# zwu88/TANTE

Measured on NVIDIA B200. Metric: training_samples_per_s, higher is better.
Workload: dtype bf16

## Files before the change

include/tante_b200.h:

```cpp
#ifndef TANTE_B200_H_
#define TANTE_B200_H_

#include <stddef.h>
#include <stdint.h>

#ifdef __cplusplus
extern "C" {
#endif

#if defined(__GNUC__)
#define TANTE_API __attribute__((visibility("default")))
#else
#define TANTE_API
#endif

#define TANTE_OK 0
#define TANTE_ERR_INVALID 1
#define TANTE_ERR_CUDA 2
#define TANTE_ERR_STATE 3
#define TANTE_ERR_NOMEM 4

#define TANTE_MAX_ORDER 8
#define TANTE_MAX_LAYERS 32

// ... 54 lines not shown
                        int32_t n_cap, float* frames, float* R_t, int32_t* n_host, void* stream);
TANTE_API int tante_backward(tante_handle_t h, int32_t slot, const float* input, const float* grad_frames,
                   int32_t n_frames, const float* grad_Rt, float* grad_input, float* grad_params, void* stream);

TANTE_API int tante_train_forward_win(tante_handle_t h, int32_t slot, const float* const* frame_ptrs,
                                      const int64_t* frame_bstride, int32_t B, float out_T, int32_t n_cap, float* frames,
                                      int64_t frames_bstride, float* R_t, int32_t* n_host, void* stream);
TANTE_API int tante_backward_win(tante_handle_t h, int32_t slot, const float* grad_frames, int64_t gf_bstride, int32_t n_frames,
                                 const float* grad_Rt, float* const* grad_frame_ptrs, const int64_t* grad_bstride,
                                 float* grad_params, void* stream);

TANTE_API int tante_train_forward_hist(tante_handle_t h, int32_t slot, const float* input, float* pred, int64_t pred_bstride,
                                       int32_t* cursor, int32_t B, float out_T, int32_t n_cap, int32_t n_steps, float* R_t,
                                       int32_t* ns, int32_t* steps, int32_t* n_active, void* stream);
TANTE_API int tante_backward_hist(tante_handle_t h, int32_t slot, float* grad_pred, int64_t gp_bstride, const float* grad_Rt,
                                  float* grad_input, float* grad_params, void* stream);

TANTE_API int tante_debug_stage(tante_handle_t h, const char* stage, float* dst, int64_t cap, int64_t* numel,
                      void* stream);
TANTE_API int64_t tante_launch_count(tante_handle_t h);

TANTE_API int tante_bench_head(tante_handle_t h, const float* u, float* frames, int32_t B, int32_t n_frames,
                     int32_t iters, float* ms_out, void* stream);

TANTE_API int tante_profile(tante_handle_t h, int32_t enable);
TANTE_API int tante_profile_read(tante_handle_t h, double* gemm_ms, double* gemm_flops, int64_t* gemm_launches);
TANTE_API int tante_profile_read_class(tante_handle_t h, int32_t cls, double* ms, double* flops, double* bytes,
                                       int64_t* launches);

TANTE_API int tante_mse_cl(const float* y, const float* ref, int32_t B, int32_t nf, int32_t n_use, int32_t D, int64_t HW,
                 int32_t n_ref, int32_t f0, float scale, const float* gout, float* loss_sum, float* grad_y, void* stream);

TANTE_API int tante_metric_moments(const float* x, const float* y, int64_t BT, int64_t HW, int32_t C, double* out,
                                   void* stream);

TANTE_API int tante_comm_unique_id(void* id128);
TANTE_API int tante_comm_init(tante_handle_t h, const void* id128, int32_t nranks, int32_t rank);
TANTE_API int tante_allreduce_grads(tante_handle_t h, float* grad, void* comm, void* stream);
TANTE_API int tante_optimizer_step(tante_handle_t h, float* grad, float* exp_avg, float* exp_avg_sq, float lr, float beta1,
                                   float beta2, float eps, float weight_decay, int64_t step, int32_t clip_mode, float clip,
                                   float grad_scale, double* grad_sumsq, void* stream);

TANTE_API int tante_test_gemm(int32_t use_tc, int32_t epi, const void* A, const void* W, const float* bias,
                    const float* resid, void* C, int32_t out_bf16, int32_t M, int32_t N, int32_t K,
                    int32_t iters, const float* ln_gamma, const float* ln_beta, void* ln_out, void* stream);

TANTE_API int tante_test_block_tail(const void* att, const void* Wo, const void* W1, const void* W2, const float* vec7,
                                    const float* x_in, float* x_out, void* ln_out, float* x_mid, void* ln2, void* hpre,
                                    void* hact, int32_t M, int32_t iters, void* stream);

TANTE_API int tante_test_wgrad(int32_t use_tc, const void* A, const void* B, float* C, float* bias, int64_t M, int32_t N,
                     int32_t K, int32_t iters, void* stream);

#ifdef __cplusplus
}
#endif
#endif
```

tante_b200/_abi.py:

```python
from __future__ import annotations

import ctypes as C
import os

_HERE = os.path.dirname(os.path.abspath(__file__))
LIB_PATH = os.path.join(_HERE, "lib", "libtante_b200.so")

TANTE_MAX_ORDER = 8
TANTE_MAX_LAYERS = 32
PREC_FP32 = 0
PREC_BF16 = 1


class TanteConfig(C.Structure):
    _fields_ = [
        ("in_T", C.c_int32), ("n_fields", C.c_int32), ("H", C.c_int32), ("W", C.c_int32),
        ("taylor_order", C.c_int32), ("n_head", C.c_int32), ("embed_dim", C.c_int32),
        ("patch_scale", C.c_int32), ("deg", C.c_int32), ("output_length", C.c_int32),
        ("frame_interval", C.c_float), ("precision", C.c_int32),
        ("n_layers", C.c_int32 * TANTE_MAX_ORDER),
        ("axes", (C.c_char * TANTE_MAX_LAYERS) * TANTE_MAX_ORDER),
        ("enc_dec_fno", C.c_int32), ("modes1", C.c_int32), ("modes2", C.c_int32),
        ("mlp_hidden", C.c_int32),
        ("expanded_channel", C.c_int32), ("mlp_hidden_c", C.c_int32),
# ... 11 lines not shown
SIGNATURES = {
    "tante_last_error": (C.c_char_p, []),
    "tante_version": (C.c_int, []),
    "tante_create": (C.c_int, [C.POINTER(TanteConfig), C.c_int, C.POINTER(C.c_void_p)]),
    "tante_destroy": (C.c_int, [C.c_void_p]),
    "tante_reserve": (C.c_int, [C.c_void_p, C.c_int32, C.c_int32, C.c_int32]),
    "tante_workspace_bytes": (C.c_int64, [C.c_void_p]),
    "tante_param_count": (C.c_int32, [C.c_void_p]),
    "tante_param_name": (C.c_char_p, [C.c_void_p, C.c_int32]),
    "tante_param_numel": (C.c_int64, [C.c_void_p, C.c_int32]),
    "tante_bind_param": (C.c_int, [C.c_void_p, C.c_char_p, C.c_void_p, C.c_void_p, C.c_int64]),
    "tante_pack_params": (C.c_int, [C.c_void_p, C.c_void_p]),
    "tante_forward": (C.c_int, [C.c_void_p, C.c_void_p, C.c_int32, C.c_float, C.c_int32, C.c_int32,
                                C.c_void_p, C.c_void_p, C.c_void_p, C.POINTER(C.c_int32), C.c_void_p]),
    "tante_rollout": (C.c_int, [C.c_void_p, C.c_void_p, C.c_int32, C.c_int32, C.c_float, C.c_int32,
                                C.c_void_p, C.c_void_p, C.c_void_p, C.c_void_p, C.c_int32, C.c_void_p]),
    "tante_debug_stage": (C.c_int, [C.c_void_p, C.c_char_p, C.c_void_p, C.c_int64, C.POINTER(C.c_int64), C.c_void_p]),
    "tante_launch_count": (C.c_int64, [C.c_void_p]),
    "tante_profile": (C.c_int, [C.c_void_p, C.c_int32]),
    "tante_profile_read": (C.c_int, [C.c_void_p, C.POINTER(C.c_double), C.POINTER(C.c_double), C.POINTER(C.c_int64)]),
    "tante_profile_read_class": (C.c_int, [C.c_void_p, C.c_int32, C.POINTER(C.c_double), C.POINTER(C.c_double),
                                           C.POINTER(C.c_double), C.POINTER(C.c_int64)]),
    "tante_mse_cl": (C.c_int, [C.c_void_p, C.c_void_p, C.c_int32, C.c_int32, C.c_int32, C.c_int32, C.c_int64, C.c_int32,
                               C.c_int32, C.c_float, C.c_void_p, C.c_void_p, C.c_void_p, C.c_void_p]),
    "tante_test_block_tail": (C.c_int, [C.c_void_p] * 12 + [C.c_int32, C.c_int32, C.c_void_p]),
    "tante_metric_moments": (C.c_int, [C.c_void_p, C.c_void_p, C.c_int64, C.c_int64, C.c_int32, C.c_void_p, C.c_void_p]),
    "tante_test_gemm": (C.c_int, [C.c_int32, C.c_int32, C.c_void_p, C.c_void_p, C.c_void_p, C.c_void_p, C.c_void_p,
                                  C.c_int32, C.c_int32, C.c_int32, C.c_int32, C.c_int32, C.c_void_p, C.c_void_p, C.c_void_p,
                                  C.c_void_p]),
    "tante_comm_unique_id": (C.c_int, [C.c_void_p]),
    "tante_comm_init": (C.c_int, [C.c_void_p, C.c_void_p, C.c_int32, C.c_int32]),
    "tante_allreduce_grads": (C.c_int, [C.c_void_p, C.c_void_p, C.c_void_p, C.c_void_p]),
    "tante_optimizer_step": (C.c_int, [C.c_void_p, C.c_void_p, C.c_void_p, C.c_void_p, C.c_float, C.c_float, C.c_float,
                                       C.c_float, C.c_float, C.c_int64, C.c_int32, C.c_float, C.c_float, C.c_void_p,
                                       C.c_void_p]),
    "tante_set_dropout": (C.c_int, [C.c_void_p, C.c_float, C.c_uint64]),
    "tante_grad_numel": (C.c_int64, [C.c_void_p]),
    "tante_param_grad_offset": (C.c_int64, [C.c_void_p, C.c_int32]),
    "tante_train_forward": (C.c_int, [C.c_void_p, C.c_int32, C.c_void_p, C.c_int32, C.c_float, C.c_int32,
                                      C.c_void_p, C.c_void_p, C.POINTER(C.c_int32), C.c_void_p]),
    "tante_backward": (C.c_int, [C.c_void_p, C.c_int32, C.c_void_p, C.c_void_p, C.c_int32, C.c_void_p, C.c_void_p,
                                 C.c_void_p, C.c_void_p]),
    "tante_train_forward_win": (C.c_int, [C.c_void_p, C.c_int32, C.POINTER(C.c_void_p), C.POINTER(C.c_int64), C.c_int32, C.c_float,
                                          C.c_int32, C.c_void_p, C.c_int64, C.c_void_p, C.POINTER(C.c_int32), C.c_void_p]),
    "tante_backward_win": (C.c_int, [C.c_void_p, C.c_int32, C.c_void_p, C.c_int64, C.c_int32, C.c_void_p, C.POINTER(C.c_void_p),
                                     C.POINTER(C.c_int64), C.c_void_p, C.c_void_p]),
    "tante_train_forward_hist": (C.c_int, [C.c_void_p, C.c_int32, C.c_void_p, C.c_void_p, C.c_int64, C.c_void_p, C.c_int32,
                                           C.c_float, C.c_int32, C.c_int32, C.c_void_p, C.c_void_p, C.c_void_p, C.c_void_p,
                                           C.c_void_p]),
    "tante_backward_hist": (C.c_int, [C.c_void_p, C.c_int32, C.c_void_p, C.c_int64, C.c_void_p, C.c_void_p, C.c_void_p,
                                      C.c_void_p]),
    "tante_test_wgrad": (C.c_int, [C.c_int32, C.c_void_p, C.c_void_p, C.c_void_p, C.c_void_p, C.c_int64, C.c_int32,
                                   C.c_int32, C.c_int32, C.c_void_p]),
    "tante_bench_head": (C.c_int, [C.c_void_p, C.c_void_p, C.c_void_p, C.c_int32, C.c_int32, C.c_int32,
                                   C.POINTER(C.c_float), C.c_void_p]),
}

_lib = None


def load() -> C.CDLL:
    global _lib
    if _lib is not None:
        return _lib
    if not os.path.exists(LIB_PATH):
        raise ImportError(
            f"{LIB_PATH} not found: build it with `python -m tante_b200.build` (nvcc, sm_100a). "
            "tante_b200 has no fallback path.")
    lib = C.CDLL(LIB_PATH)
    for name, (res, args) in SIGNATURES.items():
        fn = getattr(lib, name)
        fn.restype = res
        fn.argtypes = args
    _lib = lib
    return lib


def check(code: int):
    if code != 0:
        raise TanteError(code, (load().tante_last_error() or b"").decode())
```

tante_b200/csrc/tante_abi.cu:

```cuda
#include <cuda_runtime.h>

#include <algorithm>
#include <cmath>
#include <cstdio>
#include <cstring>
#include <map>
#include <memory>
#include <stdexcept>
#include <string>
#include <vector>

#include "../../include/tante_b200.h"
#include "common.cuh"
#include "gemm_simt.cuh"
#include "gemm_tc.cuh"
#include "attention_mma.cuh"
#include "attention_flash.cuh"
#include "propagator_mma.cuh"
#include "propagator_bwd_mma.cuh"
#include "propagator_small.cuh"
#include "head_mma.cuh"
#include "kernels_simt.cuh"
#include "pack.cuh"
#include "backward.cuh"
// ... 1288 lines not shown
template <typename TA, int ACT>
void launch_act_fwd(tante_handle_s* h, const TA* pre, TA* out, long long n, cudaStream_t st) {
    act_fwd_kernel<TA, ACT><<<blocks_for(n / 4, 256), 256, 0, st>>>(pre, out, n / 4);
    CK(cudaGetLastError());
    h->launches++;
}
template <typename TA, int ACT>
void launch_act_bwd(tante_handle_s* h, TA* g, const TA* pre, long long n, cudaStream_t st) {
    act_bwd_kernel<TA, ACT><<<blocks_for(n / 4, 256), 256, 0, st>>>(g, pre, n / 4);
    CK(cudaGetLastError());
    h->launches++;
}
template <typename TA>
void launch_colsum(tante_handle_s* h, const TA* x, int ld, long long M, int N, float* out, cudaStream_t st) {
    const unsigned gx = (unsigned)((N + 127) / 128);
    unsigned gy = (unsigned)std::max<long long>(1, std::min<long long>((M + 255) / 256, (4LL * h->num_sms + gx - 1) / gx));
    colsum_kernel<TA><<<dim3(gx, gy), 256, 0, st>>>(x, ld, M, N, out);
    CK(cudaGetLastError());
    h->launches++;
}
template <typename TA>
void wgrad(tante_handle_s* h, const TA* A, int lda, const TA* Bm, int ldb, float* out, long long M, int N, int K,
           cudaStream_t st, float* bias_out = nullptr) {
    {
        ProfScope ps(h, st, 2.0 * (double)M * N * K, 2, (double)M * (N + K) * sizeof(TA));
        if constexpr (sizeof(TA) == 2) {
            if (wgrad_tc_supported(M, N, K, K, lda, ldb, K)) {
                CK(launch_wgrad_tc(A, lda, Bm, ldb, out, K, M, N, K, K, h->num_sms, st, bias_out));
                h->launches++;
                return;
            }
        }
        CK((launch_wgrad_simt<TA, TA>(A, lda, Bm, ldb, out, K, M, N, K, h->num_sms, st)));
        h->launches++;
    }
    if (bias_out) launch_colsum<TA>(h, A, lda, M, N, bias_out, st);
}
template <typename TA>
void wgrad_pad(tante_handle_s* h, const TA* A, int lda, int N, const TA* Bm, int ldb, int Kb, float* out, int ldc, int Kc,
               long long M, cudaStream_t st, float* bias_out = nullptr) {
    {
        ProfScope ps(h, st, 2.0 * (double)M * N * Kc, 2, (double)M * (N + Kb) * sizeof(TA));
        if constexpr (sizeof(TA) == 2) {
            if (wgrad_tc_supported(M, N, Kb, Kc, lda, ldb, ldc)) {
                CK(launch_wgrad_tc(A, lda, Bm, ldb, out, ldc, M, N, Kb, Kc, h->num_sms, st, bias_out));
                h->launches++;
                return;
            }
        }
        CK((launch_wgrad_simt<TA, TA>(A, lda, Bm, ldb, out, ldc, M, N, Kc, h->num_sms, st)));
        h->launches++;
    }
    if (bias_out) launch_colsum<TA>(h, A, lda, M, N, bias_out, st);
}
template <typename TA>
void gemm_dx(tante_handle_s* h, const TA* A, int lda, int64_t wT_off, TA* out, int ldc, int M, int N, int K, cudaStream_t st) {
    EpiParams ep; ep.bias = AF(h, h->zero_off);
    REQUIRE(N <= 8192, "input-gradient GEMM wider than the zero-bias vector");
    if (sizeof(TA) == 2 && K > 1024) {
        REQUIRE(ldc == N, "input-gradient GEMM: K not covered");
        if (h->kscratch.bytes < (size_t)M * N * 4) destroy_graphs(h);
        dev_alloc(h, h->kscratch, (size_t)M * N * 4);
        float* v = FP(h->kscratch);
        gemm_bigk_f32(h, reinterpret_cast<const __nv_bfloat16*>(A), lda, wT_off, v, M, N, K, AF(h, h->zero_off), st);
        convert_kernel<TA><<<blocks_for((long long)M * N / 4, 256), 256, 0, st>>>(v, out, (long long)M * N / 4);
        CK(cudaGetLastError());
        h->launches++;
        return;
    }
    gemm<TA>(h, EPI_BIAS, A, lda, wT_off, out, ldc, sizeof(TA) == 4, M, N, K, ep, st);
}

template <typename TA, int ACT>
void gemm_dx_act(tante_handle_s* h, const TA* A, int lda, int64_t wT_off, TA* out, const TA* pre, int M, int N, int K,
                 cudaStream_t st) {
    static const bool fuse = getenv("TANTE_FUSE_ACTGRAD") && atoi(getenv("TANTE_FUSE_ACTGRAD")) != 0;
    if (sizeof(TA) == 2 && fuse) {
        EpiParams ep; ep.bias = AF(h, h->zero_off);
        REQUIRE(N <= 8192, "input-gradient GEMM wider than the zero-bias vector");
        ep.mul_pre = pre; ep.ld_pre = N;
        const int epi = ACT == ACT_RELU ? EPI_MULGRAD_RELU : (ACT == ACT_GELU_ERF ? EPI_MULGRAD_GELU_ERF : EPI_MULGRAD_GELU_TANH);
        gemm<TA>(h, epi, A, lda, wT_off, out, N, false, M, N, K, ep, st);
    } else {
        gemm_dx<TA>(h, A, lda, wT_off, out, N, M, N, K, st);
        launch_act_bwd<TA, ACT>(h, out, pre, (long long)M * N, st);
    }
}

template <typename TA>
void run_spectral_bwd(tante_handle_s* h, const SpecPlan& sp, const SpecView& x, const SpecView& g, long long N, int H, int W,
                      int level, TA* dx, float* gin, cudaStream_t st) {
    const int W0 = h->cfg.W, H0 = h->cfg.H, W1 = W0 / h->fp0;
    const float2* tw = reinterpret_cast<const float2*>(h->ftw.p);
    const float2* twW = level == 0 ? tw : tw + W0 + H0;
    const float2* twH = level == 0 ? tw + W0 : tw + W0 + H0 + W1;
    const int m1 = sp.wm1, m2 = sp.wm2, Cin = sp.Cin, Cout = sp.Cout;
    float2* A = reinterpret_cast<float2*>(h->fA.p);
    float2* Bc = reinterpret_cast<float2*>(h->fB.p);
    float2* Cc = reinterpret_cast<float2*>(h->fC.p);
    float2* Dd = reinterpret_cast<float2*>(h->fD.p);
    const long long rows_o = N * Cout * H, rows_i = N * Cin * H;
    spec_dft_w_kernel<TA><<<blocks_for(rows_o, 4), 128, 0, st>>>(g, Cout, H, W, m2, twW, A, rows_o);
    CK(cudaGetLastError());
    const long long ty = N * Cout * 2 * m1 * m2, tx = N * Cin * 2 * m1 * m2;
    spec_dft_h_kernel<<<blocks_for(ty, 256), 256, 0, st>>>(A, H, m1, m2, twH, Bc, ty);
    CK(cudaGetLastError());
// ... 869 lines not shown
        wgrad<TA>(h, dz1, N1, dmod, C, GA(h, op.decw[0]), BL, N1, C, st, GA(h, op.decb[0]));
        gemm_dx<TA>(h, dz1, N1, op.decwT[0], hd, C, BL, C, N1, st);
        }
        if (!h->cfg.deg) {
            CK(cudaMemsetAsync(h->dfilm.p, 0, (size_t)B * 2 * C * 4, st));
            {
                const int chunks = std::max(1, std::min(L, (2 * h->num_sms + B - 1) / B));
                film_apply_bwd_kernel<TA><<<dim3(B, chunks), C, 0, st>>>(hd, FP(ot.d32), FP(ot.film), dxs, FP(h->dfilm), T, L, C);
                CK(cudaGetLastError());
                h->launches++;
            }
            CK(cudaMemsetAsync(h->dcond.p, 0, (size_t)B * 4, st));
            film_bwd_kernel<<<dim3(B, 16), 256, 3 * C * sizeof(float), st>>>(
                FP(ot.rt), FP(h->dfilm), AF(h, op.mod[0]), AF(h, op.mod[1]), AF(h, op.mod[2]), AF(h, op.mod[4]),
                AF(h, op.mod[5]), AF(h, op.mod[6]), GA(h, op.mod[0]), GA(h, op.mod[1]), GA(h, op.mod[2]), GA(h, op.mod[3]),
                GA(h, op.mod[4]), GA(h, op.mod[5]), GA(h, op.mod[6]), GA(h, op.mod[7]), C, FP(h->dcond));
            CK(cudaGetLastError());
            h->launches++;
            TA* hi2 = TP<TA>(h->hi2);
            TA* hi1 = TP<TA>(h->hi1);
            interp_tail_bwd_kernel<TA><<<B, 256, (C / 4) * sizeof(float), st>>>(
                TP<TA>(ot.i2), AF(h, op.intw[2]), gRt, 1.0f / (float)K, FP(h->dcond), L, C / 4, hi2, GA(h, op.intw[2]),
                GA(h, op.intb[2]));
            CK(cudaGetLastError());
            h->launches++;
            wgrad<TA>(h, hi2, C / 4, TP<TA>(ot.i1), C / 2, GA(h, op.intw[1]), BL, C / 4, C / 2, st, GA(h, op.intb[1]));
            gemm_dx_act<TA, ACT_RELU>(h, hi2, C / 4, op.intwT[1], hi1, TP<TA>(ot.i1), BL, C / 2, C / 4, st);
            wgrad<TA>(h, hi1, C / 2, TP<TA>(ot.dl), C, GA(h, op.intw[0]), BL, C / 2, C, st, GA(h, op.intb[0]));
            gemm_dx<TA>(h, hi1, C / 2, op.intwT[0], hd, C, BL, C, C / 2, st);
        }
        add_last_frame_kernel<TA><<<blocks_for((long long)BL * C / 4, 256), 256, 0, st>>>(hd, dxs, B, T, (long long)L * C);
        CK(cudaGetLastError());
        h->launches++;
        if (mirror) {
            convert_kernel<TA><<<blocks_for((long long)tokens * C / 4, 256), 256, 0, st>>>(
                dxs, dxb, (long long)tokens * C / 4, drop, drop_site(o, (int)op.layers.size() - 1, 2));
            CK(cudaGetLastError());
            h->launches++;
        }
        TA* dxb_out = mirror ? dxb : nullptr;
        for (int li = (int)op.layers.size() - 1; li >= 0; --li) {
            const LayerPlan& lp = op.layers[li];
            const float* x_in = FP(ot.X[2 * li]);
            const float* x_mid = FP(ot.X[2 * li + 1]);
            if (lp.axis == 'C') {
                run_channel_layer_bwd<TA>(h, lp, x_in, dxs, tokens, st);
                if (mirror) {
                    convert_kernel<TA><<<blocks_for((long long)tokens * C / 4, 256), 256, 0, st>>>(dxs, dxb, (long long)tokens * C / 4);
                    CK(cudaGetLastError());
                    h->launches++;
                }
                continue;
            }
            wgrad<TA>(h, dxb, C, TP<TA>(ot.hact[li]), Hm, GA(h, lp.m2w), tokens, C, Hm, st, GA(h, lp.m2b));
            if (kTensor && h->fuse_mlp_bwd && C == kBtC && h->Hm == C) {
                {
                    ProfScope ps(h, st, 2.0 * 2.0 * tokens * C * C, 4, (double)tokens * 4 * 2 * C);
                    CK(launch_mlp_bwd(reinterpret_cast<const __nv_bfloat16*>(dxb), AH(h, lp.m2wT), AH(h, lp.m0wT),
                                      reinterpret_cast<const __nv_bfloat16*>(ot.hpre[li].p), reinterpret_cast<__nv_bfloat16*>(g1),
                                      reinterpret_cast<__nv_bfloat16*>(g2), tokens, h->num_sms, st));
                }
                h->launches++;
                wgrad<TA>(h, g1, C, TP<TA>(ot.ln2[li]), C, GA(h, lp.m0w), tokens, C, C, st, GA(h, lp.m0b));
            } else {
                gemm_dx_act<TA, ACT_GELU_TANH>(h, dxb, C, lp.m2wT, g1, TP<TA>(ot.hpre[li]), tokens, Hm, C, st);
                wgrad<TA>(h, g1, Hm, TP<TA>(ot.ln2[li]), C, GA(h, lp.m0w), tokens, Hm, C, st, GA(h, lp.m0b));
                gemm_dx<TA>(h, g1, Hm, lp.m0wT, g2, C, tokens, C, Hm, st);
            }
            launch_ln_bwd<TA>(h, g2, x_mid, lp.ln2w, dxs, dxb_out, GA(h, lp.ln2w), GA(h, lp.ln2b), tokens, st, drop,
                              drop_site(o, li, 1));
            wgrad<TA>(h, dxb, C, TP<TA>(ot.att[li]), C, GA(h, lp.outw), tokens, C, C, st, GA(h, lp.outb));
            gemm_dx<TA>(h, dxb, C, lp.outwT, g2, C, tokens, C, C, st);
            launch_attention_bwd<TA>(h, TP<TA>(ot.qkv[li]), g2, gq, B, lp.axis, st, drop, drop_site(o, li, 0));
            wgrad<TA>(h, gq, 3 * C, TP<TA>(ot.ln1[li]), C, GA(h, lp.inw), tokens, 3 * C, C, st, GA(h, lp.inb));
            gemm_dx<TA>(h, gq, 3 * C, lp.inwT, g2, C, tokens, C, 3 * C, st);
            launch_ln_bwd<TA>(h, g2, x_in, lp.ln1w, dxs, dxb_out, GA(h, lp.ln1w), GA(h, lp.ln1b), tokens, st, drop,
                              drop_site(o, std::max(li - 1, 0), 2));
        }
        const float* pin = o == 0 ? FP(ot.P[0]) : FP(tp.ord[o - 1].X.back());
        launch_propagator_bwd(h, FP(ot.P[2]), dxs, B, 2, op, st);
        launch_propagator_bwd(h, FP(ot.P[1]), dxs, B, 1, op, st);
        launch_propagator_bwd(h, pin, dxs, B, 0, op, st);
    }
    CK(cudaMemsetAsync(h->dfilm.p, 0, (size_t)T * 2 * C * 4, st));
    embed_bwd_kernel<TA><<<(L + (256 / (C / 4)) - 1) / (256 / (C / 4)), 256, 0, st>>>(dxs, FP(tp.v), AF(h, h->film_t_off), g2, FP(h->dfilm), GA(h, h->s_emb),
                                          GA(h, h->t_emb), B, T, L, C);
    CK(cudaGetLastError());
    h->launches++;
    film_bwd_kernel<<<dim3(T, 16), 256, 3 * C * sizeof(float), st>>>(
        AF(h, h->tseq_off), FP(h->dfilm), AF(h, h->tenc[0]), AF(h, h->tenc[1]), AF(h, h->tenc[2]), AF(h, h->tenc[4]),
        AF(h, h->tenc[5]), AF(h, h->tenc[6]), GA(h, h->tenc[0]), GA(h, h->tenc[1]), GA(h, h->tenc[2]), GA(h, h->tenc[3]),
        GA(h, h->tenc[4]), GA(h, h->tenc[5]), GA(h, h->tenc[6]), GA(h, h->tenc[7]), C, nullptr);
    CK(cudaGetLastError());
    h->launches++;
    const int K3 = g.k2 * g.k2 * C2, K2 = g.k1 * g.k1 * C1;
    const int M2 = tokens * g.R2;
    const long long rows_in = (long long)tokens * g.R1;
    if (h->fno) {
        TA* wb = TP<TA>(h->wbuf);
        const int H = h->cfg.H, W = h->cfg.W, p0 = h->fp0, p1 = h->fp1, H1 = H / p0, W1 = W / p0, C8 = C / 8;
        const long long NI = (long long)B * T, MF1 = NI * H1 * W1;
        const int KF2 = p1 * p1 * C2, KF1 = p0 * p0 * C8;
        TA* gr0 = TP<TA>(h->fgr0);
        TA* gr1 = TP<TA>(h->fgr1);
        TA* gr2 = TP<TA>(h->fgr2);
        auto cdimf = [](int n, int k, int sdv) { return (n + 2 * ((k - 1) / 2) - k) / sdv + 1; };
        const int Hc2 = cdimf(H1, p1, h->st[1]), Wc2 = cdimf(W1, p1, h->st[1]), Hc1 = cdimf(H, p0, h->st[0]), Wc1 = cdimf(W, p0, h->st[0]);
        const bool pool2 = Hc2 != h->Hp || Wc2 != h->Wp, pool1 = Hc1 != H1 || Wc1 != W1;
        const long long rows2 = NI * Hc2 * Wc2, rows1 = NI * Hc1 * Wc1;
        REQUIRE(rows1 < (1LL << 31) && rows2 < (1LL << 31), "input too large for the conv backward GEMMs");
        TA* cg = TP<TA>(h->cgrid);
        const TA* dY2 = g2;
        if (pool2) {
            const long long t4 = rows2 * C / 4;
            wide_pool_bwd_kernel<TA, false><<<blocks_for(t4, 256), 256, 0, st>>>(g2, nullptr, Hc2, Wc2, C, h->Hp, h->Wp, cg, t4);
            CK(cudaGetLastError());
            h->launches++;
            dY2 = cg;
        }
        wide_im2col_cl_kernel<TA><<<blocks_for(rows2 * KF2 / 4, 256), 256, 0, st>>>(TP<TA>(tp.a2act), H1, W1, C2, p1, (p1 - 1) / 2, wb,
                                                                                   rows2 * KF2 / 4, h->st[1], Hc2, Wc2);
        CK(cudaGetLastError());
        h->launches++;
        wgrad<TA>(h, dY2, C, wb, KF2, GA(h, h->enc_w[1]), rows2, C, KF2, st, GA(h, h->enc_b[1]));
        gemm_dx<TA>(h, dY2, C, h->enc_wT[1], wb, KF2, (int)rows2, KF2, C, st);
        wide_col2im_cl_kernel<TA><<<blocks_for(MF1 * C2 / 4, 256), 256, 0, st>>>(wb, H1, W1, C2, p1, (p1 - 1) / 2, gr2, MF1 * C2 / 4, h->st[1], Hc2, Wc2);
        CK(cudaGetLastError());
        h->launches++;
// ... 786 lines not shown
        win.frames_bs = pred_bstride;
        win.n_lim = n_steps;
        if (h->cfg.precision == TANTE_PREC_FP32) run_step_train<float>(h, tp, input, B, out_T, n_cap, pred, R_t, st, &win);
        else run_step_train<__nv_bfloat16>(h, tp, input, B, out_T, n_cap, pred, R_t, st, &win);
        hist_advance_kernel<<<1, 256, 0, st>>>(reinterpret_cast<const int*>(tp.n_arr.p), cursor, ns, steps, n_active, B, n_steps);
        CK(cudaGetLastError());
        h->launches++;
        h->last_B = B;
    });
}

int tante_backward_hist(tante_handle_t h, int32_t slot, float* grad_pred, int64_t gp_bstride, const float* grad_Rt,
                        float* grad_input, float* grad_params, void* stream) {
    return guarded([&] {
        REQUIRE(h && grad_pred && grad_params, "null argument");
        REQUIRE(slot >= 0 && slot < (int)h->tapes.size(), "tape slot out of range");
        REQUIRE(gp_bstride % 4 == 0, "gp_bstride must be a multiple of 4 elements");
        Tape& tp = *h->tapes[slot];
        if (!tp.valid) throw Error(TANTE_ERR_STATE, "tape slot holds no forward (or was already consumed)");
        REQUIRE(tp.hist, "tape slot was not written by tante_train_forward_hist");
        CK(cudaSetDevice(h->device));
        cudaStream_t st = reinterpret_cast<cudaStream_t>(stream);
        backward_alloc(h, tp.B_used);
        const long long DHW = (long long)h->D * h->cfg.H * h->cfg.W;
        BackwardWin win;
        win.gf_bs = gp_bstride;
        win.gin = FrameTab{};
        win.gin.on = 1;
        const long long gi = grad_input ? elem_offset(grad_input, grad_pred) : 0;
        for (int t = 0; t < h->T; ++t) {
            win.gin.off[t] = grad_input ? gi + t * DHW : kFrameSkip;
            win.gin.bs[t] = h->T * DHW;
        }
        win.gin.cur = reinterpret_cast<const int*>(tp.cur.p);
        win.gin.hoff = 0;
        win.gin.hbs = gp_bstride;
        if (h->cfg.precision == TANTE_PREC_FP32)
            run_backward<float>(h, tp, nullptr, grad_pred, tp.n_cap, grad_Rt, grad_pred, grad_params, st, &win);
        else
            run_backward<__nv_bfloat16>(h, tp, nullptr, grad_pred, tp.n_cap, grad_Rt, grad_pred, grad_params, st, &win);
        tp.valid = false;
    });
}

int tante_test_wgrad(int32_t use_tc, const void* A, const void* Bm, float* C, float* bias, int64_t M, int32_t N, int32_t K,
                     int32_t iters, void* stream) {
    return guarded([&] {
        REQUIRE(A && Bm && C, "null argument");
        cudaStream_t st = reinterpret_cast<cudaStream_t>(stream);
        int dev = 0, sms = 148;
        CK(cudaGetDevice(&dev));
        CK(cudaDeviceGetAttribute(&sms, cudaDevAttrMultiProcessorCount, dev));
        for (int i = 0; i < std::max(1, iters); ++i) {
            if (use_tc == 1) {
                const int Kb = (K + 63) / 64 * 64;
                REQUIRE(wgrad_tc_supported(M, N, Kb, K, N, Kb, K), "shape not covered by the tcgen05 wgrad kernel");
                CK(launch_wgrad_tc(reinterpret_cast<const __nv_bfloat16*>(A), N, reinterpret_cast<const __nv_bfloat16*>(Bm), Kb,
                                   C, K, M, N, Kb, K, sms, st, bias));
            } else if (use_tc == 2) {
                CK((launch_wgrad_simt<__nv_bfloat16, __nv_bfloat16>(reinterpret_cast<const __nv_bfloat16*>(A), N,
                                                                    reinterpret_cast<const __nv_bfloat16*>(Bm), K, C, K, M, N,
                                                                    K, sms, st)));
            } else {
                CK((launch_wgrad_simt<float, float>(reinterpret_cast<const float*>(A), N, reinterpret_cast<const float*>(Bm), K,
                                                    C, K, M, N, K, sms, st)));
            }
        }
    });
}

int tante_debug_stage(tante_handle_t h, const char* stage, float* dst, int64_t cap, int64_t* numel, void* stream) {
    return guarded([&] {
        REQUIRE(h && stage && dst && numel, "null argument");
        CK(cudaSetDevice(h->device));
        cudaStream_t st = reinterpret_cast<cudaStream_t>(stream);
        const std::string s(stage);
        if (s == "enable") { h->debug = true; *numel = 0; return; }
        const int B = h->last_B;
        REQUIRE(B > 0, "no forward has run yet");
        const int64_t lat = (int64_t)B * h->T * h->L * h->C;
        const void* src = nullptr;
        int64_t n = 0;
        if (s == "latent") { src = h->x.p; n = lat; }
        else if (s == "latent_in") { REQUIRE(h->debug && h->dbg_in.p, "debug capture not enabled before reserve"); src = h->dbg_in.p; n = lat; }
        else if (s == "rt") { src = h->rt.p; n = (int64_t)h->K * h->max_batch; }
        else if (s == "deriv") {
            n = (int64_t)h->K * B * h->D * h->cfg.H * h->cfg.W;
            REQUIRE(cap >= n, "destination too small");
            if (h->wide) {
                CK(cudaMemcpyAsync(dst, h->dfield.p, (size_t)n * 4, cudaMemcpyDeviceToDevice, st));
                *numel = n;
                return;
            }
            CK(cudaMemsetAsync(h->nbuf.p, 0, (size_t)B * 4, st));
            StepIO io;
            io.input = reinterpret_cast<const float*>(h->ring.p);
            RolloutState rs{};
            if (h->cfg.precision == TANTE_PREC_FP32) launch_head<float>(h, io, B, rs, dst, st);
            else launch_head<__nv_bfloat16>(h, io, B, rs, dst, st);
            *numel = n;
            return;
        }
        else throw Error(TANTE_ERR_INVALID, "unknown stage " + s);
        REQUIRE(cap >= n, "destination too small");
        CK(cudaMemcpyAsync(dst, src, (size_t)n * 4, cudaMemcpyDeviceToDevice, st));
        *numel = n;
    });
}

int64_t tante_launch_count(tante_handle_t h) { return h ? h->launches : -1; }

int tante_bench_head(tante_handle_t h, const float* u, float* frames, int32_t B, int32_t n_frames, int32_t iters,
                     float* ms_out, void* stream) {
    return guarded([&] {
        REQUIRE(h && u && frames && ms_out && n_frames >= 1 && iters >= 1, "bad argument");
        CK(cudaSetDevice(h->device));
        ensure_ready(h, B, false);
        cudaStream_t st = reinterpret_cast<cudaStream_t>(stream);
// ... 249 lines not shown
```

tante_b200/csrc/wgrad_tc.cuh:

```cuda
#pragma once
#include "gemm_tc.cuh"

namespace tante {

constexpr int kWgRows = 64;
constexpr int kWgBox = kWgRows * 128;
constexpr int kWgThreads = 192;

namespace ptx {
__device__ __forceinline__ uint64_t umma_desc_mn_sw128(uint32_t smem_addr, uint32_t lbo_bytes, uint32_t sbo_bytes) {
    return (uint64_t)((smem_addr >> 4) & 0x3FFF) | ((uint64_t)((lbo_bytes >> 4) & 0x3FFF) << 16) |
           ((uint64_t)((sbo_bytes >> 4) & 0x3FFF) << 32) | (1ull << 46) | (2ull << 61);
}
__host__ __device__ constexpr uint32_t umma_idesc_bf16_mn(int M, int N) {
    return umma_idesc_bf16(M, N) | (1u << 15) | (1u << 16);
}
__device__ __forceinline__ void bulk_load_1d(void* smem_dst, const void* gsrc, uint32_t bytes, uint64_t* bar) {
    asm volatile("cp.async.bulk.shared::cluster.global.mbarrier::complete_tx::bytes [%0], [%1], %2, [%3];"
                 ::"r"(smem_u32(smem_dst)), "l"(reinterpret_cast<uint64_t>(gsrc)), "r"(bytes), "r"(smem_u32(bar))
                 : "memory");
}
__device__ __forceinline__ void tma_reduce_add_2d(const CUtensorMap* m, const void* smem_src, int c0, int c1) {
    asm volatile("cp.reduce.async.bulk.tensor.2d.global.shared::cta.add.tile.bulk_group [%0, {%2, %3}], [%1];"
                 ::"l"(reinterpret_cast<uint64_t>(m)), "r"(smem_u32(smem_src)), "r"(c0), "r"(c1)
// ... 87 lines not shown
                        const uint64_t db = ptx::umma_desc_mn_sw128(sb + k * 2048, kWgBox, 1024);
                        ptx::umma_bf16(tmem_base, da, db, idesc, (t | k) != 0);
                        if (do_bias) {
                            uint32_t so;
                            asm volatile("mov.u32 %0, %1;" : "=r"(so) : "r"(sones));
                            ptx::umma_bf16(tmem_base + (uint32_t)BN, da, ptx::umma_desc_mn_sw128(so, kWgBox, 1024), idesc_b, (t | k) != 0);
                        }
                    }
                    ptx::umma_commit(&empty[stage]);
                    if (t == ntile - 1) ptx::umma_commit(tmem_full);
                }
                __syncwarp();
                if (++stage == nstage) { stage = 0; phase ^= 1; }
            }
        } else {
            const int q = warp & 3;
            ptx::mbar_wait(tmem_full, 0);
            ptx::tc_fence_after();
            uint8_t* buf = sStage + (size_t)(warp - 2) * kTcEpiBuf;
            const uint32_t tm = tmem_base + ((uint32_t)(q * 32) << 16);
#pragma unroll 1
            for (int ch = 0; ch < BN / 32; ++ch) {
                uint32_t r0[32];
                ptx::tmem_ld_32x32(tm + (uint32_t)(ch * 32), r0);
                if (lane == 0) ptx::bulk_wait_read<0>();
                __syncwarp();
                ptx::tc_wait_ld();
#pragma unroll
                for (int c = 0; c < 8; ++c)
                    *reinterpret_cast<uint4*>(buf + sw128_off(lane, c)) =
                        make_uint4(r0[c * 4 + 0], r0[c * 4 + 1], r0[c * 4 + 2], r0[c * 4 + 3]);
                ptx::fence_proxy_async();
                __syncwarp();
                if (lane == 0) {
                    ptx::tma_reduce_add_2d(&tmC, buf, k0 + ch * 32, n0 + q * 32);
                    ptx::bulk_commit();
                }
            }
            if (do_bias) {
                uint32_t r0[32];
                ptx::tmem_ld_32x32(tm + (uint32_t)BN, r0);
                ptx::tc_wait_ld();
                const int n = n0 + q * 32 + lane;
                if (n < n_total) atomicAdd(bias_grad + n, __uint_as_float(r0[0]));
            }
            if (lane == 0) ptx::bulk_wait_all<0>();
        }
    }
    ptx::tc_fence_before();
    __syncthreads();
    if (warp == 1) ptx::tmem_dealloc(tmem_base, kTmemCols);
}

static cudaError_t wg_set_attrs() {
    static unsigned long long done = 0;
    if (!attrs_needed(done)) return cudaSuccess;
    cudaError_t e;
    if ((e = cudaFuncSetAttribute(wgrad_tc_kernel<256>, cudaFuncAttributeMaxDynamicSharedMemorySize, 227 * 1024)) != cudaSuccess) return e;
    if ((e = cudaFuncSetAttribute(wgrad_tc_kernel<128>, cudaFuncAttributeMaxDynamicSharedMemorySize, 227 * 1024)) != cudaSuccess) return e;
    if ((e = cudaFuncSetAttribute(wgrad_tc_kernel<64>, cudaFuncAttributeMaxDynamicSharedMemorySize, 227 * 1024)) != cudaSuccess) return e;
    return cudaSuccess;
}

static const __nv_bfloat16* wg_ones(cudaError_t* err) {
    static void* ptr[64] = {nullptr};
    int dev = 0;
    if ((*err = cudaGetDevice(&dev)) != cudaSuccess) return nullptr;
    if (dev < 0 || dev >= 64) { *err = cudaErrorInvalidDevice; return nullptr; }
    if (!ptr[dev]) {
        uint16_t host[kWgBox / 2];
        for (int i = 0; i < kWgBox / 2; ++i) host[i] = 0x3F80;
        void* p = nullptr;
        if ((*err = cudaMalloc(&p, kWgBox)) != cudaSuccess) return nullptr;
        if ((*err = cudaMemcpy(p, host, kWgBox, cudaMemcpyHostToDevice)) != cudaSuccess) return nullptr;
        ptr[dev] = p;
    }
    return reinterpret_cast<const __nv_bfloat16*>(ptr[dev]);
}

static bool wgrad_tc_supported(long long M, int N, int Kb, int Kc, int lda, int ldb, int ldc) {
    return M >= 64 && M < (1LL << 31) && N % 64 == 0 && Kb % 64 == 0 && Kc <= Kb && Kc >= 1 && lda % 8 == 0 &&
           ldb % 8 == 0 && ldc % 4 == 0;
}

static cudaError_t launch_wgrad_tc(const __nv_bfloat16* A, int lda, const __nv_bfloat16* Bm, int ldb, float* Cout,
                                   int ldc, long long M, int N, int Kb, int Kc, int num_sms, cudaStream_t st,
                                   float* bias_grad = nullptr) {
    if (!wgrad_tc_supported(M, N, Kb, Kc, lda, ldb, ldc)) return cudaErrorInvalidValue;
    const int BN = (Kb % 256 == 0) ? 256 : (Kb % 128 == 0 ? 128 : 64);
    const int stage_bytes = (2 + BN / 64) * kWgBox;
    int nstage = (int)((227 * 1024 - 2048 - kWgBox) / stage_bytes);
    nstage = nstage > 6 ? 6 : nstage;
    const size_t smem = (size_t)nstage * stage_bytes + kWgBox + 256 + 1024;
    const int m_tiles = (int)((M + kWgRows - 1) / kWgRows);
    const int n_tiles = (N + 127) / 128;
    const int tiles_xy = n_tiles * (Kb / BN);
    int splits = std::max(1, num_sms / tiles_xy);
    splits = std::min(splits, m_tiles);
    const int per = (m_tiles + splits - 1) / splits;
    splits = (m_tiles + per - 1) / per;
    CUtensorMap tmA, tmB, tmC;
    if (!make_tmap_2d(&tmA, CU_TENSOR_MAP_DATA_TYPE_BFLOAT16, 2, A, (int)M, N, lda, 64, kWgRows)) return cudaErrorInvalidValue;
    if (!make_tmap_2d(&tmB, CU_TENSOR_MAP_DATA_TYPE_BFLOAT16, 2, Bm, (int)M, Kb, ldb, 64, kWgRows)) return cudaErrorInvalidValue;
    if (!make_tmap_2d(&tmC, CU_TENSOR_MAP_DATA_TYPE_FLOAT32, 4, Cout, N, Kc, ldc, 32, 32)) return cudaErrorInvalidValue;
    { cudaError_t e = wg_set_attrs(); if (e != cudaSuccess) return e; }
    const __nv_bfloat16* ones = nullptr;
    if (bias_grad) { cudaError_t e = cudaSuccess; ones = wg_ones(&e); if (e != cudaSuccess) return e; }
    cudaLaunchConfig_t cfg = {};
    cfg.gridDim = dim3(n_tiles, Kb / BN, splits); cfg.blockDim = dim3(kWgThreads); cfg.dynamicSmemBytes = smem; cfg.stream = st;
    cudaLaunchAttribute at[1];
    int na = 0;
    if (pdl_enabled(st)) {
        at[na].id = cudaLaunchAttributeProgrammaticStreamSerialization;
        at[na].val.programmaticStreamSerializationAllowed = 1;
        ++na;
    }
    cfg.attrs = at; cfg.numAttrs = (unsigned)na;
    switch (BN) {
        case 256: return cudaLaunchKernelEx(&cfg, wgrad_tc_kernel<256>, tmA, tmB, tmC, m_tiles, per, nstage, bias_grad, N, ones);
        case 128: return cudaLaunchKernelEx(&cfg, wgrad_tc_kernel<128>, tmA, tmB, tmC, m_tiles, per, nstage, bias_grad, N, ones);
        default: return cudaLaunchKernelEx(&cfg, wgrad_tc_kernel<64>, tmA, tmB, tmC, m_tiles, per, nstage, bias_grad, N, ones);
    }
}

}
```

Measured before the change: 623.8.

## Add CTA-pair tcgen05 grouped wgrad kernel and batch per-layer weight gradients

Adds a 2-CTA cluster wgrad kernel using paired UMMA with 256x256 tiles, covering up to four problems in one grouped launch. Each split accumulates into fp32 outputs via TMA reduce-add, and bias gradients are computed alongside. The backward pass now batches the MLP wgrads, and the out-proj and in-proj wgrads, into single grouped launches, with the in-proj pair moved after the dx GEMM. The aim is fewer launches, better SM fill on small weight GEMMs, and more operand reuse per tile. The cost is more complex cluster synchronisation and larger tiles that only apply when N and K are multiples of 256.

```diff
diff --git a/include/tante_b200.h b/include/tante_b200.h
--- a/include/tante_b200.h
+++ b/include/tante_b200.h
@@ -130,6 +130,10 @@
 TANTE_API int tante_test_wgrad(int32_t use_tc, const void* A, const void* B, float* C, float* bias, int64_t M, int32_t N,
                      int32_t K, int32_t iters, void* stream);
 
+TANTE_API int tante_test_wgrad_group(int32_t grouped, int32_t nprob, const void* const* A, const void* const* B,
+                                     float* const* C, float* const* bias, const int32_t* N, const int32_t* K, int64_t M,
+                                     int32_t iters, void* stream);
+
 #ifdef __cplusplus
 }
 #endif
diff --git a/tante_b200/_abi.py b/tante_b200/_abi.py
--- a/tante_b200/_abi.py
+++ b/tante_b200/_abi.py
@@ -87,6 +87,9 @@
                                       C.c_void_p]),
     "tante_test_wgrad": (C.c_int, [C.c_int32, C.c_void_p, C.c_void_p, C.c_void_p, C.c_void_p, C.c_int64, C.c_int32,
                                    C.c_int32, C.c_int32, C.c_void_p]),
+    "tante_test_wgrad_group": (C.c_int, [C.c_int32, C.c_int32, C.POINTER(C.c_void_p), C.POINTER(C.c_void_p),
+                                         C.POINTER(C.c_void_p), C.POINTER(C.c_void_p), C.POINTER(C.c_int32),
+                                         C.POINTER(C.c_int32), C.c_int64, C.c_int32, C.c_void_p]),
     "tante_bench_head": (C.c_int, [C.c_void_p, C.c_void_p, C.c_void_p, C.c_int32, C.c_int32, C.c_int32,
                                    C.POINTER(C.c_float), C.c_void_p]),
 }
diff --git a/tante_b200/csrc/tante_abi.cu b/tante_b200/csrc/tante_abi.cu
--- a/tante_b200/csrc/tante_abi.cu
+++ b/tante_b200/csrc/tante_abi.cu
@@ -1364,6 +1364,31 @@
         h->launches++;
     }
     if (bias_out) launch_colsum<TA>(h, A, lda, M, N, bias_out, st);
+}
+template <typename TA>
+struct WgradArgs { const TA* A; int lda; const TA* Bm; int ldb; float* out; int N, K; float* bias_out; };
+template <typename TA>
+void wgrad_group(tante_handle_s* h, std::initializer_list<WgradArgs<TA>> args, long long M, cudaStream_t st) {
+    if constexpr (sizeof(TA) == 2) {
+        WgradProblem pr[kWgMaxProblems];
+        int n = 0;
+        bool ok = args.size() <= (size_t)kWgMaxProblems;
+        double flops = 0.0, bytes = 0.0;
+        for (const WgradArgs<TA>& a : args) {
+            if (!ok) break;
+            pr[n] = {a.A, a.lda, a.Bm, a.ldb, a.out, a.K, a.N, a.K, a.K, a.bias_out};
+            ok = wgrad_pair_supported(M, pr[n++]);
+            flops += 2.0 * (double)M * a.N * a.K;
+            bytes += (double)M * (a.N + a.K) * sizeof(TA);
+        }
+        if (ok) {
+            ProfScope ps(h, st, flops, 2, bytes);
+            CK(launch_wgrad_group(pr, n, M, h->num_sms, st));
+            h->launches++;
+            return;
+        }
+    }
+    for (const WgradArgs<TA>& a : args) wgrad<TA>(h, a.A, a.lda, a.Bm, a.ldb, a.out, M, a.N, a.K, st, a.bias_out);
 }
 template <typename TA>
 void gemm_dx(tante_handle_s* h, const TA* A, int lda, int64_t wT_off, TA* out, int ldc, int M, int N, int K, cudaStream_t st) {
@@ -2339,7 +2364,6 @@
                 }
                 continue;
             }
-            wgrad<TA>(h, dxb, C, TP<TA>(ot.hact[li]), Hm, GA(h, lp.m2w), tokens, C, Hm, st, GA(h, lp.m2b));
             if (kTensor && h->fuse_mlp_bwd && C == kBtC && h->Hm == C) {
                 {
                     ProfScope ps(h, st, 2.0 * 2.0 * tokens * C * C, 4, (double)tokens * 4 * 2 * C);
@@ -2348,19 +2372,27 @@
                                       reinterpret_cast<__nv_bfloat16*>(g2), tokens, h->num_sms, st));
                 }
                 h->launches++;
-                wgrad<TA>(h, g1, C, TP<TA>(ot.ln2[li]), C, GA(h, lp.m0w), tokens, C, C, st, GA(h, lp.m0b));
+                wgrad_group<TA>(h, {{dxb, C, TP<TA>(ot.hact[li]), Hm, GA(h, lp.m2w), C, Hm, GA(h, lp.m2b)},
+                                    {g1, C, TP<TA>(ot.ln2[li]), C, GA(h, lp.m0w), C, C, GA(h, lp.m0b)}},
+                                tokens, st);
             } else {
+                wgrad<TA>(h, dxb, C, TP<TA>(ot.hact[li]), Hm, GA(h, lp.m2w), tokens, C, Hm, st, GA(h, lp.m2b));
                 gemm_dx_act<TA, ACT_GELU_TANH>(h, dxb, C, lp.m2wT, g1, TP<TA>(ot.hpre[li]), tokens, Hm, C, st);
                 wgrad<TA>(h, g1, Hm, TP<TA>(ot.ln2[li]), C, GA(h, lp.m0w), tokens, Hm, C, st, GA(h, lp.m0b));
                 gemm_dx<TA>(h, g1, Hm, lp.m0wT, g2, C, tokens, C, Hm, st);
             }
             launch_ln_bwd<TA>(h, g2, x_mid, lp.ln2w, dxs, dxb_out, GA(h, lp.ln2w), GA(h, lp.ln2b), tokens, st, drop,
                               drop_site(o, li, 1));
-            wgrad<TA>(h, dxb, C, TP<TA>(ot.att[li]), C, GA(h, lp.outw), tokens, C, C, st, GA(h, lp.outb));
+            if (!kTensor) wgrad<TA>(h, dxb, C, TP<TA>(ot.att[li]), C, GA(h, lp.outw), tokens, C, C, st, GA(h, lp.outb));
             gemm_dx<TA>(h, dxb, C, lp.outwT, g2, C, tokens, C, C, st);
             launch_attention_bwd<TA>(h, TP<TA>(ot.qkv[li]), g2, gq, B, lp.axis, st, drop, drop_site(o, li, 0));
-            wgrad<TA>(h, gq, 3 * C, TP<TA>(ot.ln1[li]), C, GA(h, lp.inw), tokens, 3 * C, C, st, GA(h, lp.inb));
+            if (!kTensor) wgrad<TA>(h, gq, 3 * C, TP<TA>(ot.ln1[li]), C, GA(h, lp.inw), tokens, 3 * C, C, st, GA(h, lp.inb));
             gemm_dx<TA>(h, gq, 3 * C, lp.inwT, g2, C, tokens, C, 3 * C, st);
+            if (kTensor) {
+                wgrad_group<TA>(h, {{dxb, C, TP<TA>(ot.att[li]), C, GA(h, lp.outw), C, C, GA(h, lp.outb)},
+                                    {gq, 3 * C, TP<TA>(ot.ln1[li]), C, GA(h, lp.inw), 3 * C, C, GA(h, lp.inb)}},
+                                tokens, st);
+            }
             launch_ln_bwd<TA>(h, g2, x_in, lp.ln1w, dxs, dxb_out, GA(h, lp.ln1w), GA(h, lp.ln1b), tokens, st, drop,
                               drop_site(o, std::max(li - 1, 0), 2));
         }
@@ -3253,11 +3285,15 @@
         CK(cudaGetDevice(&dev));
         CK(cudaDeviceGetAttribute(&sms, cudaDevAttrMultiProcessorCount, dev));
         for (int i = 0; i < std::max(1, iters); ++i) {
-            if (use_tc == 1) {
+            if (use_tc == 1 || use_tc == 3) {
                 const int Kb = (K + 63) / 64 * 64;
                 REQUIRE(wgrad_tc_supported(M, N, Kb, K, N, Kb, K), "shape not covered by the tcgen05 wgrad kernel");
-                CK(launch_wgrad_tc(reinterpret_cast<const __nv_bfloat16*>(A), N, reinterpret_cast<const __nv_bfloat16*>(Bm), Kb,
-                                   C, K, M, N, Kb, K, sms, st, bias));
+                if (use_tc == 1)
+                    CK(launch_wgrad_tc(reinterpret_cast<const __nv_bfloat16*>(A), N, reinterpret_cast<const __nv_bfloat16*>(Bm), Kb,
+                                       C, K, M, N, Kb, K, sms, st, bias));
+                else
+                    CK(launch_wgrad_single(reinterpret_cast<const __nv_bfloat16*>(A), N, reinterpret_cast<const __nv_bfloat16*>(Bm),
+                                           Kb, C, K, M, N, Kb, K, sms, st, bias));
             } else if (use_tc == 2) {
                 CK((launch_wgrad_simt<__nv_bfloat16, __nv_bfloat16>(reinterpret_cast<const __nv_bfloat16*>(A), N,
                                                                     reinterpret_cast<const __nv_bfloat16*>(Bm), K, C, K, M, N,
@@ -3265,6 +3301,34 @@
             } else {
                 CK((launch_wgrad_simt<float, float>(reinterpret_cast<const float*>(A), N, reinterpret_cast<const float*>(Bm), K,
                                                     C, K, M, N, K, sms, st)));
+            }
+        }
+    });
+}
+
+int tante_test_wgrad_group(int32_t grouped, int32_t nprob, const void* const* A, const void* const* B, float* const* C,
+                           float* const* bias, const int32_t* N, const int32_t* K, int64_t M, int32_t iters, void* stream) {
+    return guarded([&] {
+        REQUIRE(A && B && C && bias && N && K, "null argument");
+        REQUIRE(nprob >= 1 && nprob <= kWgMaxProblems, "nprob must be 1..4");
+        cudaStream_t st = reinterpret_cast<cudaStream_t>(stream);
+        int dev = 0, sms = 148;
+        CK(cudaGetDevice(&dev));
+        CK(cudaDeviceGetAttribute(&sms, cudaDevAttrMultiProcessorCount, dev));
+        WgradProblem pr[kWgMaxProblems];
+        for (int i = 0; i < nprob; ++i) {
+            REQUIRE(A[i] && B[i] && C[i], "null argument");
+            pr[i] = {reinterpret_cast<const __nv_bfloat16*>(A[i]), N[i], reinterpret_cast<const __nv_bfloat16*>(B[i]), K[i],
+                     C[i], K[i], N[i], K[i], K[i], bias[i]};
+            REQUIRE(wgrad_pair_supported(M, pr[i]), "shape not covered by the CTA-pair wgrad kernel");
+        }
+        for (int it = 0; it < std::max(1, iters); ++it) {
+            if (grouped) {
+                CK(launch_wgrad_group(pr, nprob, M, sms, st));
+            } else {
+                for (int i = 0; i < nprob; ++i)
+                    CK(launch_wgrad_single(pr[i].A, pr[i].lda, pr[i].B, pr[i].ldb, pr[i].C, pr[i].ldc, M, pr[i].N, pr[i].Kb,
+                                           pr[i].Kc, sms, st, pr[i].bias));
             }
         }
     });
diff --git a/tante_b200/csrc/wgrad_tc.cuh b/tante_b200/csrc/wgrad_tc.cuh
--- a/tante_b200/csrc/wgrad_tc.cuh
+++ b/tante_b200/csrc/wgrad_tc.cuh
@@ -163,10 +163,169 @@
     if (warp == 1) ptx::tmem_dealloc(tmem_base, kTmemCols);
 }
 
+constexpr int kWgMaxProblems = 4;
+constexpr int kWgPairStage = 4 * kWgBox;
+constexpr int kWgPairBufs = 8;
+
+struct WgGroup {
+    CUtensorMap a[kWgMaxProblems];
+    CUtensorMap b[kWgMaxProblems];
+    CUtensorMap c[kWgMaxProblems];
+    CUtensorMap ones;
+    float* bias[kWgMaxProblems];
+    int n_tiles[kWgMaxProblems];
+    int tile_end[kWgMaxProblems];
+    int nprob, m_tiles, splits, nstage;
+};
+
+__global__ void __launch_bounds__(kWgThreads, 1) __cluster_dims__(2, 1, 1)
+wgrad_pair_kernel(const __grid_constant__ WgGroup g) {
+    pdl_trigger();
+    extern __shared__ uint8_t smem_raw[];
+    uint8_t* smem = smem_raw + ((1024u - (ptx::smem_u32(smem_raw) & 1023u)) & 1023u);
+    uint8_t* sOnes = smem;
+    uint8_t* sStage = smem + kWgBox;
+    uint64_t* bars = reinterpret_cast<uint64_t*>(sStage + (size_t)g.nstage * kWgPairStage);
+    uint64_t* full = bars;
+    uint64_t* empty = bars + 8;
+    uint64_t* tmem_full = bars + 16;
+    uint64_t* ones_full = bars + 17;
+    uint32_t* tmem_slot = reinterpret_cast<uint32_t*>(bars + 18);
+    constexpr int kTmemCols = 512;
+
+    const int warp = threadIdx.x / 32, lane = threadIdx.x % 32;
+    const int crank = (int)ptx::cluster_ctarank();
+    const int cid = blockIdx.x / 2;
+    const int tile = cid / g.splits, split = cid % g.splits;
+    int p = 0;
+    while (p + 1 < g.nprob && tile >= g.tile_end[p]) ++p;
+    const int lt = tile - (p ? g.tile_end[p - 1] : 0);
+    const int n0 = (lt % g.n_tiles[p]) * 256, k0 = (lt / g.n_tiles[p]) * 256;
+    const int t_begin = (int)((long long)split * g.m_tiles / g.splits);
+    const int t_end = (int)((long long)(split + 1) * g.m_tiles / g.splits);
+    const int ntile = t_end - t_begin;
+    float* bias_grad = k0 == 0 ? g.bias[p] : nullptr;
+    const CUtensorMap* tmA = &g.a[p];
+    const CUtensorMap* tmB = &g.b[p];
+    const CUtensorMap* tmC = &g.c[p];
+
+    if (warp == 0 && lane == 0) {
+        ptx::prefetch_tmap(tmA);
+        ptx::prefetch_tmap(tmB);
+        ptx::prefetch_tmap(tmC);
+        for (int s = 0; s < g.nstage; ++s) { ptx::mbar_init(&full[s], 1); ptx::mbar_init(&empty[s], 1); }
+        ptx::mbar_init(tmem_full, 1);
+        ptx::mbar_init(ones_full, 1);
+        ptx::fence_barrier_init();
+    }
+    if (warp == 1) {
+        ptx::tmem_alloc_pair(tmem_slot, kTmemCols);
+        ptx::tmem_relinquish_pair();
+    }
+    ptx::tc_fence_before();
+    ptx::cluster_sync_all();
+    ptx::tc_fence_after();
+    const uint32_t tmem_base = *tmem_slot;
+    pdl_wait();
+
+    if (ntile > 0) {
+        if (warp == 0) {
+            if (lane == 0) {
+                if (bias_grad) {
+                    if (crank == 0) ptx::mbar_arrive_expect_tx(ones_full, 2 * kWgBox);
+                    ptx::tma_load_2d_pair(sOnes, &g.ones, ones_full, 0, 0);
+                }
+                int stage = 0;
+                uint32_t phase = 0;
+                for (int t = t_begin; t < t_end; ++t) {
+                    ptx::mbar_wait(&empty[stage], phase ^ 1);
+                    if (crank == 0) ptx::mbar_arrive_expect_tx(&full[stage], 2 * kWgPairStage);
+                    uint8_t* sa = sStage + (size_t)stage * kWgPairStage;
+                    uint8_t* sb = sa + 2 * kWgBox;
+                    const int nc = n0 + crank * 128, kc = k0 + crank * 128;
+                    ptx::tma_load_2d_pair(sa, tmA, &full[stage], nc, t * kWgRows);
+                    ptx::tma_load_2d_pair(sa + kWgBox, tmA, &full[stage], nc + 64, t * kWgRows);
+                    ptx::tma_load_2d_pair(sb, tmB, &full[stage], kc, t * kWgRows);
+                    ptx::tma_load_2d_pair(sb + kWgBox, tmB, &full[stage], kc + 64, t * kWgRows);
+                    if (++stage == g.nstage) { stage = 0; phase ^= 1; }
+                }
+            }
+        } else if (warp == 1) {
+            if (crank == 0) {
+                constexpr uint32_t idesc = ptx::umma_idesc_bf16_mn(256, 256);
+                constexpr uint32_t idesc_b = ptx::umma_idesc_bf16_mn(256, 128);
+                const uint32_t sones = ptx::smem_u32(sOnes);
+                int stage = 0;
+                uint32_t phase = 0;
+                if (bias_grad) ptx::mbar_wait(ones_full, 0);
+                for (int t = 0; t < ntile; ++t) {
+                    ptx::mbar_wait(&full[stage], phase);
+                    ptx::tc_fence_after();
+                    if (lane == 0) {
+                        const uint32_t sa = ptx::smem_u32(sStage + (size_t)stage * kWgPairStage);
+                        const uint32_t sb = sa + 2 * kWgBox;
+#pragma unroll
+                        for (int k = 0; k < kWgRows / 16; ++k) {
+                            const uint64_t da = ptx::umma_desc_mn_sw128(sa + k * 2048, kWgBox, 1024);
+                            const uint64_t db = ptx::umma_desc_mn_sw128(sb + k * 2048, kWgBox, 1024);
+                            ptx::umma_bf16_pair(tmem_base, da, db, idesc, (t | k) != 0);
+                            if (bias_grad) {
+                                uint32_t so;
+                                asm volatile("mov.u32 %0, %1;" : "=r"(so) : "r"(sones));
+                                ptx::umma_bf16_pair(tmem_base + 256u, da, ptx::umma_desc_mn_sw128(so, kWgBox, 1024), idesc_b,
+                                                    (t | k) != 0);
+                            }
+                        }
+                        ptx::umma_commit_pair(&empty[stage]);
+                        if (t == ntile - 1) ptx::umma_commit_pair(tmem_full);
+                    }
+                    __syncwarp();
+                    if (++stage == g.nstage) { stage = 0; phase ^= 1; }
+                }
+            }
+        } else {
+            const int q = warp & 3;
+            const int row0 = n0 + crank * 128 + q * 32;
+            ptx::mbar_wait(tmem_full, 0);
+            ptx::tc_fence_after();
+            uint8_t* ebuf = sStage + (size_t)(warp - 2) * kWgPairBufs * kTcEpiBuf;
+            const uint32_t tm = tmem_base + ((uint32_t)(q * 32) << 16);
+#pragma unroll 1
+            for (int ch = 0; ch < 256 / 32; ++ch) {
+                uint32_t r0[32];
+                ptx::tmem_ld_32x32(tm + (uint32_t)(ch * 32), r0);
+                ptx::tc_wait_ld();
+                uint8_t* buf = ebuf + ch * kTcEpiBuf;
+#pragma unroll
+                for (int c = 0; c < 8; ++c)
+                    *reinterpret_cast<uint4*>(buf + sw128_off(lane, c)) =
+                        make_uint4(r0[c * 4 + 0], r0[c * 4 + 1], r0[c * 4 + 2], r0[c * 4 + 3]);
+                ptx::fence_proxy_async();
+                __syncwarp();
+                if (lane == 0) {
+                    ptx::tma_reduce_add_2d(tmC, buf, k0 + ch * 32, row0);
+                    ptx::bulk_commit();
+                }
+            }
+            if (bias_grad) {
+                uint32_t r0[32];
+                ptx::tmem_ld_32x32(tm + 256u, r0);
+                ptx::tc_wait_ld();
+                atomicAdd(bias_grad + row0 + lane, __uint_as_float(r0[0]));
+            }
+            if (lane == 0) ptx::bulk_wait_all<0>();
+        }
+    }
+    ptx::tc_fence_before();
+    ptx::cluster_sync_all();
+    if (warp == 1) ptx::tmem_dealloc_pair(tmem_base, kTmemCols);
+}
+
 static cudaError_t wg_set_attrs() {
     static unsigned long long done = 0;
     if (!attrs_needed(done)) return cudaSuccess;
     cudaError_t e;
+    if ((e = cudaFuncSetAttribute(wgrad_pair_kernel, cudaFuncAttributeMaxDynamicSharedMemorySize, 227 * 1024)) != cudaSuccess) return e;
     if ((e = cudaFuncSetAttribute(wgrad_tc_kernel<256>, cudaFuncAttributeMaxDynamicSharedMemorySize, 227 * 1024)) != cudaSuccess) return e;
     if ((e = cudaFuncSetAttribute(wgrad_tc_kernel<128>, cudaFuncAttributeMaxDynamicSharedMemorySize, 227 * 1024)) != cudaSuccess) return e;
     if ((e = cudaFuncSetAttribute(wgrad_tc_kernel<64>, cudaFuncAttributeMaxDynamicSharedMemorySize, 227 * 1024)) != cudaSuccess) return e;
@@ -194,9 +353,65 @@
            ldb % 8 == 0 && ldc % 4 == 0;
 }
 
-static cudaError_t launch_wgrad_tc(const __nv_bfloat16* A, int lda, const __nv_bfloat16* Bm, int ldb, float* Cout,
-                                   int ldc, long long M, int N, int Kb, int Kc, int num_sms, cudaStream_t st,
-                                   float* bias_grad = nullptr) {
+struct WgradProblem {
+    const __nv_bfloat16* A; int lda;
+    const __nv_bfloat16* B; int ldb;
+    float* C; int ldc;
+    int N, Kb, Kc;
+    float* bias;
+};
+
+static bool wgrad_pair_supported(long long M, const WgradProblem& p) {
+    return wgrad_tc_supported(M, p.N, p.Kb, p.Kc, p.lda, p.ldb, p.ldc) && p.N % 256 == 0 && p.Kb % 256 == 0;
+}
+
+static cudaError_t launch_wgrad_group(const WgradProblem* probs, int nprob, long long M, int num_sms, cudaStream_t st) {
+    if (nprob < 1 || nprob > kWgMaxProblems) return cudaErrorInvalidValue;
+    WgGroup g;
+    memset(&g, 0, sizeof(g));
+    int tiles = 0;
+    for (int i = 0; i < nprob; ++i) {
+        const WgradProblem& p = probs[i];
+        if (!wgrad_pair_supported(M, p)) return cudaErrorInvalidValue;
+        if (!make_tmap_2d(&g.a[i], CU_TENSOR_MAP_DATA_TYPE_BFLOAT16, 2, p.A, (int)M, p.N, p.lda, 64, kWgRows)) return cudaErrorInvalidValue;
+        if (!make_tmap_2d(&g.b[i], CU_TENSOR_MAP_DATA_TYPE_BFLOAT16, 2, p.B, (int)M, p.Kb, p.ldb, 64, kWgRows)) return cudaErrorInvalidValue;
+        if (!make_tmap_2d(&g.c[i], CU_TENSOR_MAP_DATA_TYPE_FLOAT32, 4, p.C, p.N, p.Kc, p.ldc, 32, 32)) return cudaErrorInvalidValue;
+        g.bias[i] = p.bias;
+        g.n_tiles[i] = p.N / 256;
+        tiles += (p.N / 256) * (p.Kb / 256);
+        g.tile_end[i] = tiles;
+    }
+    bool any_bias = false;
+    for (int i = 0; i < nprob; ++i) any_bias |= probs[i].bias != nullptr;
+    if (any_bias) {
+        cudaError_t e = cudaSuccess;
+        const __nv_bfloat16* ones = wg_ones(&e);
+        if (e != cudaSuccess) return e;
+        if (!make_tmap_2d(&g.ones, CU_TENSOR_MAP_DATA_TYPE_BFLOAT16, 2, ones, 64, 64, 64, 64, 64)) return cudaErrorInvalidValue;
+    }
+    g.nprob = nprob;
+    g.m_tiles = (int)((M + kWgRows - 1) / kWgRows);
+    g.splits = std::max(1, std::min(g.m_tiles, (num_sms / 2) / tiles));
+    g.nstage = std::min(6, (int)((227 * 1024 - 1024 - 256 - kWgBox) / kWgPairStage));
+    if (g.nstage * kWgPairStage < 4 * kWgPairBufs * kTcEpiBuf) return cudaErrorInvalidValue;
+    const size_t smem = (size_t)g.nstage * kWgPairStage + kWgBox + 256 + 1024;
+    { cudaError_t e = wg_set_attrs(); if (e != cudaSuccess) return e; }
+    cudaLaunchConfig_t cfg = {};
+    cfg.gridDim = dim3(2u * (unsigned)(tiles * g.splits)); cfg.blockDim = dim3(kWgThreads); cfg.dynamicSmemBytes = smem; cfg.stream = st;
+    cudaLaunchAttribute at[1];
+    int na = 0;
+    if (pdl_enabled(st)) {
+        at[na].id = cudaLaunchAttributeProgrammaticStreamSerialization;
+        at[na].val.programmaticStreamSerializationAllowed = 1;
+        ++na;
+    }
+    cfg.attrs = at; cfg.numAttrs = (unsigned)na;
+    return cudaLaunchKernelEx(&cfg, wgrad_pair_kernel, g);
+}
+
+static cudaError_t launch_wgrad_single(const __nv_bfloat16* A, int lda, const __nv_bfloat16* Bm, int ldb, float* Cout,
+                                       int ldc, long long M, int N, int Kb, int Kc, int num_sms, cudaStream_t st,
+                                       float* bias_grad = nullptr) {
     if (!wgrad_tc_supported(M, N, Kb, Kc, lda, ldb, ldc)) return cudaErrorInvalidValue;
     const int BN = (Kb % 256 == 0) ? 256 : (Kb % 128 == 0 ? 128 : 64);
     const int stage_bytes = (2 + BN / 64) * kWgBox;
@@ -234,4 +449,12 @@
     }
 }
 
-}
+static cudaError_t launch_wgrad_tc(const __nv_bfloat16* A, int lda, const __nv_bfloat16* Bm, int ldb, float* Cout,
+                                   int ldc, long long M, int N, int Kb, int Kc, int num_sms, cudaStream_t st,
+                                   float* bias_grad = nullptr) {
+    const WgradProblem p = {A, lda, Bm, ldb, Cout, ldc, N, Kb, Kc, bias_grad};
+    if (wgrad_pair_supported(M, p)) return launch_wgrad_group(&p, 1, M, num_sms, st);
+    return launch_wgrad_single(A, lda, Bm, ldb, Cout, ldc, M, N, Kb, Kc, num_sms, st, bias_grad);
+}
+
+}
```

After: 632.8, median of 6. 1.01x the previous value.
